# Improbable-AI/walk-these-ways

Hardware: NVIDIA H100
Metric: env_steps_per_s (higher is better)
Workload: dtype tf32

## Files before the change

### walk-these-ways_b200/csrc/gemm_tf32.cu

```cuda
#include <cuda_runtime.h>
#include <cuda.h>
#include <stdint.h>
#include <stdio.h>
#include <mutex>
#include <unordered_map>
#include <stdlib.h>
#include "../../include/go1_b200.h"
#include "wgmma_tf32.cuh"
#include "activation.cuh"

extern int go1_set_error(const char* m);
void go1_count_launch(int n);

namespace {

constexpr int BM = 128, BK = 32;
constexpr int NCONS = 8, EPI_G = 2;

__device__ __forceinline__ uint32_t smem_u32(const void* p) { return (uint32_t)__cvta_generic_to_shared(p); }

__device__ __forceinline__ void mbar_init(uint64_t* bar, uint32_t count) {
    asm volatile("mbarrier.init.shared::cta.b64 [%0], %1;" ::"r"(smem_u32(bar)), "r"(count));
}
__device__ __forceinline__ void mbar_expect_tx(uint64_t* bar, uint32_t bytes) {
    asm volatile("mbarrier.arrive.expect_tx.shared::cta.b64 _, [%0], %1;" ::"r"(smem_u32(bar)), "r"(bytes) : "memory");
}
__device__ __forceinline__ void mbar_wait(uint64_t* bar, uint32_t parity) {
    uint32_t done = 0;
    const uint32_t a = smem_u32(bar);
    while (!done) {
        asm volatile("{\n\t.reg .pred p;\n\tmbarrier.try_wait.parity.shared::cta.b64 p, [%1], %2;\n\tselp.u32 %0, 1, 0, p;\n\t}"
                     : "=r"(done) : "r"(a), "r"(parity) : "memory");
    }
}
__device__ __forceinline__ void mbar_arrive(uint64_t* bar) {
    asm volatile("mbarrier.arrive.shared::cta.b64 _, [%0];" ::"r"(smem_u32(bar)) : "memory");
}
__device__ __forceinline__ bool elect_one() {
    uint32_t pred = 0;
    asm volatile("{\n\t.reg .pred p;\n\telect.sync _|p, 0xffffffff;\n\tselp.u32 %0, 1, 0, p;\n\t}" : "=r"(pred));
    return pred != 0;
}
__device__ __forceinline__ void tma_load_2d(const CUtensorMap* map, uint64_t* bar, void* dst, int c0, int c1) {
    asm volatile("cp.async.bulk.tensor.2d.shared::cluster.global.mbarrier::complete_tx::bytes [%0], [%1, {%3, %4}], [%2];"
                 ::"r"(smem_u32(dst)), "l"(map), "r"(smem_u32(bar)), "r"(c0), "r"(c1) : "memory");
}
__device__ __forceinline__ void cons_sync() { asm volatile("bar.sync 1, 256;" ::: "memory"); }
__device__ __forceinline__ void wg_sync(int wgi) { asm volatile("bar.sync %0, 128;" ::"r"(2 + wgi) : "memory"); }
__device__ __forceinline__ void fence_async_smem() { asm volatile("fence.proxy.async.shared::cta;" ::: "memory"); }

template <int W>
__device__ __forceinline__ void transpose_tile(const float* __restrict__ raw, uint8_t* dst, const int ctid) {
#pragma unroll
    for (int it = 0; it < W * 8 / 256; it++) {
        const int idx = ctid + 256 * it;
        const int mn = idx % W, kq = idx / W;
        const float* r = raw + (size_t)(4 * kq) * W + mn;
        *reinterpret_cast<float4*>(dst + mn * 128 + ((kq ^ (mn & 7)) << 4)) = make_float4(r[0], r[W], r[2 * W], r[3 * W]);
    }
}

template <int NJ, typename F>
__device__ __forceinline__ void store_fragment(const float (&acc)[4 * NJ], uint8_t* tile, const int col_base, const int w, const int lane, F f) {
    const int rb = 16 * w + (lane >> 2);
#pragma unroll
    for (int j = 0; j < NJ; j++) {
        const int col = col_base + 8 * j + 2 * (lane & 3);
        uint8_t* p = tile + (size_t)(col >> 5) * (64 * 128) + rb * 128 + ((((col & 31) >> 2) ^ (rb & 7)) << 4) + (lane & 1) * 8;
        *reinterpret_cast<float2*>(p) = f(make_float2(acc[4 * j], acc[4 * j + 1]), col, 0);
        *reinterpret_cast<float2*>(p + 8 * 128) = f(make_float2(acc[4 * j + 2], acc[4 * j + 3]), col, 1);
    }
}


struct GemmArgs {
    float* C; const float* bias;
    int M, N, K, ldc, act, kind, accumulate, kb_per_split;
    const float* ex; const float* wex; const float* aux;
    int ldex, ldwex, nex, ldaux;
    int lead;
    int amn, bmn;
    int ct;
    float* colsum;
    const float* bx; const float* bwx; float* gwx; float* dx;
    int ldbx, ldbwx, ldgwx, lddx, nbx;
    int tma_store, tma_aux;
    float* Cg[4]; int nprob, tiles_per_prob;
};
constexpr int GEMM_MAXP = 4;
struct GemmMaps { CUtensorMap a[GEMM_MAXP], b[GEMM_MAXP]; };

struct EpiStage {
    uint8_t* out;
    const CUtensorMap* mapC;
    const uint8_t* aux;
};
__device__ __forceinline__ void tma_store_2d(const CUtensorMap* map, const void* src, int c0, int c1) {
    asm volatile("cp.async.bulk.tensor.2d.global.shared::cta.bulk_group [%0, {%2, %3}], [%1];"
                 ::"l"(map), "r"(smem_u32(src)), "r"(c0), "r"(c1) : "memory");
}

template <typename D>
__device__ __forceinline__ void epilogue_dact(const D dact, const GemmArgs& g, float (&v)[32], const int row, const int col0, const int ncols, const int lane,
                                              const float4 (&ypre)[8], const bool have_pre, const EpiStage& es) {
    const float* arow = g.aux + (size_t)row * g.ldaux + col0;
    if (es.aux) {
        const uint8_t* srow = es.aux + lane * 128;
#pragma unroll
        for (int j = 0; j < 8; j++) {
            const float4 y = *reinterpret_cast<const float4*>(srow + ((j ^ (lane & 7)) << 4));
            v[4 * j] *= dact(y.x); v[4 * j + 1] *= dact(y.y); v[4 * j + 2] *= dact(y.z); v[4 * j + 3] *= dact(y.w);
        }
    } else if (have_pre) {
#pragma unroll
        for (int j = 0; j < 8; j++) {
            const float4 y = ypre[j];
            v[4 * j] *= dact(y.x); v[4 * j + 1] *= dact(y.y); v[4 * j + 2] *= dact(y.z); v[4 * j + 3] *= dact(y.w);
        }
    } else if (ncols == 32 && (g.ldaux & 3) == 0 && ((((uintptr_t)g.aux) & 15) == 0) && ((col0 & 3) == 0)) {
#pragma unroll
        for (int j = 0; j < 8; j++) {
            const float4 y = __ldg(reinterpret_cast<const float4*>(arow) + j);
            v[4 * j] *= dact(y.x); v[4 * j + 1] *= dact(y.y); v[4 * j + 2] *= dact(y.z); v[4 * j + 3] *= dact(y.w);
        }
    } else {
#pragma unroll
        for (int j = 0; j < 32; j++) if (j < ncols) v[j] *= dact(__ldg(arow + j));
    }
}

__device__ __forceinline__ float transpose_reduce32(float (&sred)[32], const int lane) {
#pragma unroll
    for (int off = 16; off >= 1; off >>= 1) {
        const bool upper = (lane & off) != 0;
#pragma unroll
        for (int j = 0; j < off; j++) {
            const float send = upper ? sred[j] : sred[j + off];
            const float keep = upper ? sred[j + off] : sred[j];
            sred[j] = keep + __shfl_xor_sync(0xffffffffu, send, off);
        }
    }
    return sred[0];
}
// ... 92 lines not shown
                const float s = transpose_reduce32(sred, lane);
                if (lane < ncols) atomicAdd(g.gwx + (size_t)cjx * g.ldgwx + t, s);
                }
                if (g.dx) {
                    const float wl = lane < ncols ? __ldg(g.bwx + (size_t)cjx * g.ldbwx + t) : 0.f;
                    float acc = 0.f;
#pragma unroll
                    for (int j = 0; j < 32; j++) acc = fmaf(v[j], __shfl_sync(0xffffffffu, wl, j), acc);
                    if (row_ok) atomicAdd(g.dx + (size_t)row * g.lddx + t, acc);
                }
            }
        }
    }
    if (es.out) {
        if (g.ct) {
            __syncwarp();
#pragma unroll
            for (int j = 0; j < 32; j++)
                *reinterpret_cast<float*>(es.out + j * 128 + ((((lane >> 2) ^ (j & 7)) << 4) | ((lane & 3) << 2))) = v[j];
        } else {
            uint8_t* srow = es.out + lane * 128;
#pragma unroll
            for (int j = 0; j < 8; j++)
                *reinterpret_cast<float4*>(srow + ((j ^ (lane & 7)) << 4)) = make_float4(v[4 * j], v[4 * j + 1], v[4 * j + 2], v[4 * j + 3]);
        }
        asm volatile("fence.proxy.async.shared::cta;" ::: "memory");
        __syncwarp();
        if (lane == 0) {
            if (g.ct) tma_store_2d(es.mapC, es.out, row, col0);
            else tma_store_2d(es.mapC, es.out, col0, row);
            asm volatile("cp.async.bulk.commit_group;" ::: "memory");
        }
        return;
    }
    if (!row_ok) return;
    if (vec) {
#pragma unroll
        for (int j = 0; j < 8; j++) reinterpret_cast<float4*>(crow)[j] = make_float4(v[4 * j], v[4 * j + 1], v[4 * j + 2], v[4 * j + 3]);
    } else {
#pragma unroll
        for (int j = 0; j < 32; j++) if (j < ncols) crow[j] = v[j];
    }
}

__device__ __forceinline__ bool epilogue_prefetch(const GemmArgs& g, const int row, const int col0, const bool split, float4 (&ypre)[8]) {
    if (g.act != 2 || split || col0 + 32 > g.N || (g.ldaux & 3) != 0 || ((((uintptr_t)g.aux) & 15) != 0) || (col0 & 3) != 0) return false;
    const float4* arow = reinterpret_cast<const float4*>(g.aux + (size_t)(row < g.M ? row : 0) * g.ldaux + col0);
#pragma unroll
    for (int j = 0; j < 8; j++) ypre[j] = __ldg(arow + j);
    return true;
}

constexpr int X_BYTES = 65536;
template <int BN, bool ANYKIND>
__global__ void __launch_bounds__(32 * NCONS + 128, 1) gemm_tf32_wgmma(const __grid_constant__ GemmMaps gm,
                                                                      const __grid_constant__ CUtensorMap mapC, const __grid_constant__ CUtensorMap mapY, const GemmArgs g,
                                                                      const int tiles_m, const int tiles_n, const int total_tiles, const int stages) {
    constexpr int G = EPI_G;
    constexpr int A_BYTES = BM * BK * 4, STAGE_BYTES = (BM + BN) * BK * 4;
    constexpr int MAX_STAGES = 8;
    extern __shared__ __align__(1024) uint8_t smem_raw[];
    uint8_t* base = (uint8_t*)(((uintptr_t)smem_raw + 1023) & ~(uintptr_t)1023);
    uint8_t* ring = base;
    uint8_t* xreg = base + (size_t)stages * STAGE_BYTES;
    uint8_t* stage_aux = xreg + X_BYTES;
    uint64_t* full = (uint64_t*)(stage_aux + (g.tma_aux ? NCONS * 4096 : 0));
    uint64_t* empty = full + MAX_STAGES;
    uint64_t* aux_bar = empty + MAX_STAGES;

    const int warp = threadIdx.x >> 5, lane = threadIdx.x & 31;
    const int num_kb_total = (g.K + BK - 1) / BK;

    if (threadIdx.x == 0) {
        for (int p = 0; p < g.nprob; p++) {
            asm volatile("prefetch.tensormap [%0];" ::"l"(&gm.a[p]) : "memory");
            asm volatile("prefetch.tensormap [%0];" ::"l"(&gm.b[p]) : "memory");
        }
        if (g.tma_store) asm volatile("prefetch.tensormap [%0];" ::"l"(&mapC) : "memory");
        if (g.tma_aux) asm volatile("prefetch.tensormap [%0];" ::"l"(&mapY) : "memory");
        for (int s = 0; s < stages; s++) { mbar_init(&full[s], 1); mbar_init(&empty[s], NCONS); }
        for (int w = 0; w < NCONS; w++) mbar_init(&aux_bar[w], 1);
        asm volatile("fence.mbarrier_init.release.cluster;" ::: "memory");
    }
    __syncthreads();

    auto tile_coords = [&](int t, int& m0, int& n0, int& kb0, int& nkb) {
        if (g.nprob > 1) t %= g.tiles_per_prob;
        const int tn = t % tiles_n; t /= tiles_n;
        const int tm = t % tiles_m; const int z = t / tiles_m;
        m0 = tm * BM; n0 = tn * BN; kb0 = z * g.kb_per_split; nkb = min(g.kb_per_split, num_kb_total - kb0);
    };

    if (warp == NCONS) {
        if (elect_one()) {
            int s = 0, ph = 0;
            for (int t = blockIdx.x; t < total_tiles; t += gridDim.x) {
                int m0, n0, kb0, nkb; tile_coords(t, m0, n0, kb0, nkb);
                const int p = g.nprob > 1 ? t / g.tiles_per_prob : 0;
                const CUtensorMap* mapA = &gm.a[p];
                const CUtensorMap* mapB = &gm.b[p];
                for (int i = 0; i < nkb; i++) {
                    mbar_wait(&empty[s], ph ^ 1);
                    mbar_expect_tx(&full[s], STAGE_BYTES);
                    uint8_t* a = ring + (size_t)s * STAGE_BYTES;
                    uint8_t* b = a + A_BYTES;
                    if (g.amn) tma_load_2d(mapA, &full[s], a, m0, (kb0 + i) * BK);
                    else tma_load_2d(mapA, &full[s], a, (kb0 + i) * BK, m0);
                    if (g.bmn) tma_load_2d(mapB, &full[s], b, n0, (kb0 + i) * BK);
                    else tma_load_2d(mapB, &full[s], b, (kb0 + i) * BK, n0);
                    if (++s == stages) { s = 0; ph ^= 1; }
                }
            }
        }
        return;
    }
    if (warp > NCONS) return;

    const int wgi = warp >> 2, w = warp & 3, ctid = threadIdx.x;
    const int q = 2 * wgi + (w & 1), grp = w >> 1;
    const bool tr = g.amn || g.bmn;
    const bool split = g.kb_per_split < num_kb_total;
    const bool st_out = g.tma_store, st_aux = g.tma_aux;
    uint8_t* xwg = xreg + wgi * (X_BYTES / 2);
    uint8_t* my_aux = stage_aux + warp * 4096;
    uint64_t* my_bar = &aux_bar[warp];
    int pt = blockIdx.x, pc = grp - G;
    auto next_chunk = [&]() -> bool {
        for (;;) {
            pc += G;
            if (pc >= BN / 32) { pt += gridDim.x; pc = grp; }
            if (pt >= total_tiles) return false;
            if (pc < BN / 32 && (pt % tiles_n) * BN + 32 * pc < g.N) return true;
        }
    };
    auto request_aux = [&]() {
        if (next_chunk() && lane == 0) {
            int m0, n0, kb0, nkb; tile_coords(pt, m0, n0, kb0, nkb);
            mbar_expect_tx(my_bar, 4096);
            tma_load_2d(&mapY, my_bar, my_aux, n0 + 32 * pc, m0 + 32 * q);
        }
    };
    if (st_aux) request_aux();
    uint32_t aux_phase = 0;
    int s = 0, ph = 0;
    float acc[BN / 2];
    for (int t = blockIdx.x; t < total_tiles; t += gridDim.x) {
        int m0, n0, kb0, nkb; tile_coords(t, m0, n0, kb0, nkb);
        if (st_out && lane == 0) asm volatile("cp.async.bulk.wait_group.read 0;" ::: "memory");
        cons_sync();
        int prev = -1;
        for (int i = 0; i < nkb; i++) {
            mbar_wait(&full[s], ph);
            const uint8_t* a = ring + (size_t)s * STAGE_BYTES;
            const uint8_t* b = a + A_BYTES;
            if (tr) {
                if (g.amn) { uint8_t* ta = xreg + (i & 1) * A_BYTES; transpose_tile<BM>((const float*)a, ta, ctid); a = ta; }
                if (g.bmn) { uint8_t* tb = xreg + 2 * A_BYTES + (i & 1) * A_BYTES; transpose_tile<BN>((const float*)b, tb, ctid); b = tb; }
                if (prev >= 0) {
                    wg::wait<0>();
                    if (lane == 0) mbar_arrive(&empty[prev]);
                }
                fence_async_smem();
                cons_sync();
            }
            wg::fence();
            wg::mma_kblock<BN>(acc, a + (size_t)wgi * 64 * 128, b, i > 0);
            wg::commit();
            if (!tr && prev >= 0) {
                wg::wait<1>();
                if (lane == 0) mbar_arrive(&empty[prev]);
            }
            prev = s;
            if (++s == stages) { s = 0; ph ^= 1; }
        }
        wg::wait<0>();
        if (lane == 0) mbar_arrive(&empty[prev]);
        if (tr) cons_sync();

        const int row = m0 + 32 * q + lane;
        float* const Cbase = g.nprob > 1 ? g.Cg[t / g.tiles_per_prob] : g.C;
        float4 ypre[8];
        const bool have_pre = !st_aux && (grp < BN / 32) && epilogue_prefetch(g, row, n0 + 32 * grp, split, ypre);
        store_fragment<BN / 8>(acc, xwg, 0, w, lane, [](float2 v, int, int) { return v; });
        wg_sync(wgi);
#pragma unroll 1
        for (int c = grp; c < BN / 32; c += G) {
            if (n0 + 32 * c >= g.N) break;
            uint8_t* blk = xwg + (size_t)c * (64 * 128) + (w & 1) * 4096;
            uint32_t r[32];
            const uint8_t* srow = blk + lane * 128;
#pragma unroll
            for (int j = 0; j < 8; j++) {
                const uint4 x = *reinterpret_cast<const uint4*>(srow + ((j ^ (lane & 7)) << 4));
                r[4 * j] = x.x; r[4 * j + 1] = x.y; r[4 * j + 2] = x.z; r[4 * j + 3] = x.w;
            }
            EpiStage es;
            es.out = st_out ? blk : nullptr; es.mapC = &mapC; es.aux = st_aux ? my_aux : nullptr;
            if (st_aux) { mbar_wait(my_bar, aux_phase); aux_phase ^= 1; }
            epilogue_chunk<ANYKIND>(g, Cbase, r, row, n0 + 32 * c, split, lane, ypre, have_pre && c == grp, es);
            if (st_aux) { __syncwarp(); request_aux(); }
        }
    }
    if (st_out && lane == 0) asm volatile("cp.async.bulk.wait_group 0;" ::: "memory");
}

typedef CUresult (*EncodeTiledFn)(CUtensorMap*, CUtensorMapDataType, cuuint32_t, void*, const cuuint64_t*, const cuuint64_t*, const cuuint32_t*,
                                  const cuuint32_t*, CUtensorMapInterleave, CUtensorMapSwizzle, CUtensorMapL2promotion, CUtensorMapFloatOOBfill);
EncodeTiledFn g_encode = nullptr;
std::once_flag g_once;

int sm_count() {
    static int sms = 0;
    if (!sms) { int dev = 0; cudaGetDevice(&dev); cudaDeviceGetAttribute(&sms, cudaDevAttrMultiProcessorCount, dev); if (sms <= 0) sms = 132; }
    return sms;
}

int make_map_uncached(CUtensorMap* map, const float* ptr, int rows, int cols, int ld, int box_rows, int box_cols, CUtensorMapSwizzle swz);
struct MapKey { const float* ptr; int rows, cols, ld, box_rows, box_cols, swz; bool operator==(const MapKey& o) const { return ptr == o.ptr && rows == o.rows && cols == o.cols && ld == o.ld && box_rows == o.box_rows && box_cols == o.box_cols && swz == o.swz; } };
struct MapKeyHash { size_t operator()(const MapKey& k) const { size_t h = (size_t)k.ptr; h = h * 1000003u ^ (size_t)k.rows; h = h * 1000003u ^ (size_t)k.cols; h = h * 1000003u ^ (size_t)k.ld; h = h * 1000003u ^ (size_t)(k.box_rows * 8 + k.swz); h = h * 1000003u ^ (size_t)k.box_cols; return h; } };
std::unordered_map<MapKey, CUtensorMap, MapKeyHash> g_map_cache;
std::mutex g_map_mutex;
int make_map(CUtensorMap* map, const float* ptr, int rows, int cols, int ld, int box_rows, int box_cols = BK, CUtensorMapSwizzle swz = CU_TENSOR_MAP_SWIZZLE_128B) {
    const MapKey key{ptr, rows, cols, ld, box_rows, box_cols, (int)swz};
    {
        std::lock_guard<std::mutex> lk(g_map_mutex);
        auto it = g_map_cache.find(key);
        if (it != g_map_cache.end()) { *map = it->second; return 0; }
    }
    if (int e = make_map_uncached(map, ptr, rows, cols, ld, box_rows, box_cols, swz)) return e;
    std::lock_guard<std::mutex> lk(g_map_mutex);
    if (g_map_cache.size() > 8192) g_map_cache.clear();
    g_map_cache.emplace(key, *map);
    return 0;
}
int make_map_mn(CUtensorMap* map, const float* ptr, int k_rows, int mn_cols, int ld, int width) {
    return make_map(map, ptr, k_rows, mn_cols, ld, BK, width, CU_TENSOR_MAP_SWIZZLE_NONE);
}
int make_map_uncached(CUtensorMap* map, const float* ptr, int rows, int cols, int ld, int box_rows, int box_cols, CUtensorMapSwizzle swz) {
    std::call_once(g_once, [] {
        void* fn = nullptr;
        cudaDriverEntryPointQueryResult q;
        if (cudaGetDriverEntryPoint("cuTensorMapEncodeTiled", &fn, cudaEnableDefault, &q) == cudaSuccess && q == cudaDriverEntryPointSuccess) g_encode = (EncodeTiledFn)fn;
    });
    if (!g_encode) return go1_set_error("cuTensorMapEncodeTiled unavailable");
    cuuint64_t dims[2] = {(cuuint64_t)cols, (cuuint64_t)rows};
    cuuint64_t strides[1] = {(cuuint64_t)ld * 4};
    cuuint32_t box[2] = {(cuuint32_t)box_cols, (cuuint32_t)box_rows};
    cuuint32_t estr[2] = {1, 1};
    CUresult r = g_encode(map, CU_TENSOR_MAP_DATA_TYPE_FLOAT32, 2, (void*)ptr, dims, strides, box, estr, CU_TENSOR_MAP_INTERLEAVE_NONE,
                          swz, CU_TENSOR_MAP_L2_PROMOTION_L2_256B, CU_TENSOR_MAP_FLOAT_OOB_FILL_NONE);
    if (r != CUDA_SUCCESS) { char b[96]; snprintf(b, sizeof b, "cuTensorMapEncodeTiled failed (%d)", (int)r); return go1_set_error(b); }
    return 0;
}

int split_count(int tiles, int num_kb, int min_kb, int sms) {
    constexpr int SPLIT_TILE_KB = 4;
    int best = 1;
    long long best_cost = -1;
    for (int s = 1; s <= num_kb / (min_kb > 0 ? min_kb : 1); s++) {
        const int kb = (num_kb + s - 1) / s;
        if ((num_kb + kb - 1) / kb != s) continue;
        const long long cost = (long long)(((long long)tiles * s + sms - 1) / sms) * (kb + SPLIT_TILE_KB);
        if (best_cost < 0 || cost < best_cost) { best = s; best_cost = cost; }
    }
    return best;
}

__global__ void zero_strided(float* C, int ldc, int M, int N) {
    const size_t i = (size_t)blockIdx.x * blockDim.x + threadIdx.x;
    if (i >= (size_t)M * N) return;
    C[(i / N) * ldc + (i % N)] = 0.f;
}
__global__ void bias_act_strided(float* C, int ldc, const float* bias, int M, int N, int act, int kind) {
    const size_t i = (size_t)blockIdx.x * blockDim.x + threadIdx.x;
    if (i >= (size_t)M * N) return;
    float* c = C + (i / N) * ldc + (i % N);
    float v = *c;
    if (bias) v += bias[i % N];
    if (act == 1) { GO1_ACT_SWITCH(kind, KD, v = act_exact<KD>(v);) }
    *c = v;
}

template <int BN, bool ANYKIND>
int launch_gemm(const GemmMaps& gm, const CUtensorMap& mc, const CUtensorMap& my, GemmArgs& g, int splits, cudaStream_t st) {
    constexpr int STAGE_BYTES = (BM + BN) * BK * 4;
    const size_t staging = X_BYTES + (g.tma_aux ? (size_t)NCONS * 4096 : 0);
    const size_t fixed = staging + (2 * 8 + NCONS) * 8 + 16 + 1024;
    const size_t budget = 227 * 1024;
    int stages = (int)((budget - fixed) / STAGE_BYTES);
    if (stages > 8) stages = 8;
    if (stages < 2) return go1_set_error("go1_gemm impl=1: no room for the operand ring");
    const size_t smem = (size_t)stages * STAGE_BYTES + fixed;
    static bool configured = false;
    if (!configured) {
        cudaError_t e = cudaFuncSetAttribute(gemm_tf32_wgmma<BN, ANYKIND>, cudaFuncAttributeMaxDynamicSharedMemorySize, (int)budget);
        if (e != cudaSuccess) return go1_set_error(cudaGetErrorString(e));
        configured = true;
    }
    const int tiles_m = (g.M + BM - 1) / BM, tiles_n = (g.N + BN - 1) / BN;
    g.tiles_per_prob = tiles_m * tiles_n * splits;
    const int total = g.tiles_per_prob * (g.nprob > 1 ? g.nprob : 1);
    const int sms = sm_count();
    const int grid = total < sms ? total : sms;
    gemm_tf32_wgmma<BN, ANYKIND><<<grid, 32 * NCONS + 128, smem, st>>>(gm, mc, my, g, tiles_m, tiles_n, total, stages);
    go1_count_launch(1);
    return 0;
}

constexpr int TAIL_MAXP = 2, TAIL_HPW = 12, TAIL_BM = 64;
struct TailProb { const float* b2; const float* b3; const float* Wh; const float* bh; float* y3; float* out; int ldy3, ldout, nh, wh_row0; };
struct TailArgs { TailProb p[TAIL_MAXP]; int nprob, M, tiles_per_prob, tiles, kind; };
struct TailMaps { CUtensorMap x[TAIL_MAXP], w2[TAIL_MAXP], w3[TAIL_MAXP], y2[TAIL_MAXP]; };

template <int K1, int N2, int N3>
struct TailSmem {
    static constexpr int S1 = (N3 > 0) ? 2 : 3, S2 = (N3 > 0) ? 2 : 0;
    static constexpr int KB1 = K1 / BK, KB2 = N2 / BK;
    static constexpr int STAGE1 = (TAIL_BM + N2) * BK * 4;
    static constexpr int Y2TILE = KB2 * TAIL_BM * BK * 4;
    static constexpr int STAGE2 = (N3 > 0 ? N3 : 8) * BK * 4;
    static constexpr int NL = (N3 > 0) ? N3 : N2;
    static constexpr int PARAMS = (TAIL_MAXP * (N2 + N3) + 16 * NL + TAIL_MAXP * 16) * 4;
    static constexpr int HP = TAIL_HPW * TAIL_BM * 4;
    static constexpr int BARS = (2 * S1 + 2 * (S2 > 0 ? S2 : 1)) * 8 + 16;
    static constexpr int TOTAL = S1 * STAGE1 + Y2TILE + S2 * STAGE2 + PARAMS + HP + BARS + 1024;
};

template <int NJ>
__device__ __forceinline__ void head_partial(const float (&v)[4 * NJ], const float* wh, const int NL, const int nh, const int col_base, const int lane, float (&hp)[2][TAIL_HPW]) {
#pragma unroll
    for (int n = 0; n < TAIL_HPW; n++) {
        if (n < nh) {
            const float* wr = wh + n * NL + col_base + 2 * (lane & 3);
            float a0 = hp[0][n], a1 = hp[1][n];
#pragma unroll
            for (int j = 0; j < NJ; j++) {
                const float2 ww = *reinterpret_cast<const float2*>(wr + 8 * j);
                a0 = fmaf(v[4 * j], ww.x, a0); a0 = fmaf(v[4 * j + 1], ww.y, a0);
                a1 = fmaf(v[4 * j + 2], ww.x, a1); a1 = fmaf(v[4 * j + 3], ww.y, a1);
            }
            hp[0][n] = a0; hp[1][n] = a1;
        }
    }
}

template <int K1, int N2, int N3, bool ANYKIND>
__global__ void __launch_bounds__(32 * NCONS + 128, 1) mlp_tail_fwd_kernel(const __grid_constant__ TailMaps maps, const TailArgs g) {
    const int kind = ANYKIND ? g.kind : (int)GO1_ACT_ELU;
    using L = TailSmem<K1, N2, N3>;
    constexpr int S1 = L::S1, S2 = (L::S2 > 0 ? L::S2 : 1), KB1 = L::KB1, KB2 = L::KB2, STAGE1 = L::STAGE1, STAGE2 = L::STAGE2, NL = L::NL;
    constexpr int NH2 = N2 / 2, NH3 = (N3 > 0 ? N3 : 64) / 2;
    extern __shared__ __align__(1024) uint8_t smem_raw[];
    uint8_t* base = (uint8_t*)(((uintptr_t)smem_raw + 1023) & ~(uintptr_t)1023);
    uint8_t* r1 = base;
    uint8_t* y2t = r1 + S1 * STAGE1;
    uint8_t* r2 = y2t + L::Y2TILE;
    float* s_b2 = (float*)(r2 + L::S2 * STAGE2);
// ... 130 lines not shown
            if (n < pr.nh) {
#pragma unroll
                for (int r = 0; r < 2; r++) {
                    float a = hp[r][n];
                    a += __shfl_xor_sync(0xffffffffu, a, 1);
                    a += __shfl_xor_sync(0xffffffffu, a, 2);
                    hp[r][n] = a;
                }
                if (wgi == 1 && (lane & 3) == 0) { s_hp[n * TAIL_BM + rA] = hp[0][n]; s_hp[n * TAIL_BM + rA + 8] = hp[1][n]; }
            }
        }
        cons_sync();
        if (wgi == 0 && (lane & 3) == 0) {
            const float* bh = s_bh + p * 16;
#pragma unroll
            for (int n = 0; n < TAIL_HPW; n++) {
                if (n < pr.nh) {
                    if (ok0) pr.out[(size_t)(m0 + rA) * pr.ldout + n] = hp[0][n] + s_hp[n * TAIL_BM + rA] + bh[n];
                    if (ok1) pr.out[(size_t)(m0 + rA + 8) * pr.ldout + n] = hp[1][n] + s_hp[n * TAIL_BM + rA + 8] + bh[n];
                }
            }
        }
        if (lane == 0) asm volatile("cp.async.bulk.wait_group.read 0;" ::: "memory");
        cons_sync();
    }
    if (lane == 0) asm volatile("cp.async.bulk.wait_group 0;" ::: "memory");
}

template <int K1, int N2, int N3, bool ANYKIND>
int launch_tail(const TailMaps& maps, const TailArgs& g, cudaStream_t st) {
    using L = TailSmem<K1, N2, N3>;
    static_assert(L::TOTAL <= 227 * 1024, "fused tail: shared memory budget");
    const size_t smem = L::TOTAL;
    static bool configured = false;
    if (!configured) {
        cudaError_t e = cudaFuncSetAttribute(mlp_tail_fwd_kernel<K1, N2, N3, ANYKIND>, cudaFuncAttributeMaxDynamicSharedMemorySize, (int)smem);
        if (e != cudaSuccess) return go1_set_error(cudaGetErrorString(e));
        configured = true;
    }
    const int sms = sm_count();
    const int grid = g.tiles < sms ? g.tiles : sms;
    mlp_tail_fwd_kernel<K1, N2, N3, ANYKIND><<<grid, 32 * NCONS + 128, smem, st>>>(maps, g);
    go1_count_launch(1);
    return 0;
}

}

#include <vector>
static bool g_time_on = false;
static std::vector<cudaEvent_t> g_time_events;
static size_t g_time_used = 0;
static double g_time_flop = 0.0;
struct TimeRec { int M, N, K, amn, bmn, act, nex, splits, kern, colsum; };
static std::vector<TimeRec> g_time_recs;
static cudaEvent_t timing_event() {
    if (g_time_used == g_time_events.size()) { cudaEvent_t e; cudaEventCreate(&e); g_time_events.push_back(e); }
    return g_time_events[g_time_used++];
}
extern "C" int go1_gemm_timing(int on, double* total_ms, double* total_flop, long long* launches) {
    if (on) { g_time_on = true; g_time_used = 0; g_time_flop = 0.0; g_time_recs.clear(); return 0; }
    g_time_on = false;
    double ms = 0.0;
    FILE* csv = getenv("GO1_GEMM_TIMING_CSV") ? fopen(getenv("GO1_GEMM_TIMING_CSV"), "w") : nullptr;
    if (csv) fprintf(csv, "M,N,K,a_mn_major,b_mn_major,act,num_extra,splits,kernel,colsum,us\n");
    for (size_t i = 0; i + 1 < g_time_used; i += 2) {
        if (cudaEventSynchronize(g_time_events[i + 1]) != cudaSuccess) return go1_set_error("go1_gemm_timing: event sync failed");
        float t = 0.f;
        if (cudaEventElapsedTime(&t, g_time_events[i], g_time_events[i + 1]) != cudaSuccess) return go1_set_error("go1_gemm_timing: elapsed time failed");
        ms += t;
        if (csv && i / 2 < g_time_recs.size()) {
            const TimeRec& r = g_time_recs[i / 2];
            fprintf(csv, "%d,%d,%d,%d,%d,%d,%d,%d,%s,%d,%.2f\n", r.M, r.N, r.K, r.amn, r.bmn, r.act, r.nex, r.splits,
                    r.kern >= 1000 ? (r.kern == 1003 ? "tail3" : "tail2") : (r.kern == 128 ? "p128" : (r.kern == 64 ? "p64" : "p32")), r.colsum, 1e3 * t);
        }
    }
    if (csv) fclose(csv);
    if (total_ms) *total_ms = ms;
    if (total_flop) *total_flop = g_time_flop;
    if (launches) *launches = (long long)(g_time_used / 2);
    return 0;
}

static int gemm_tf32_impl(int transA, int transB, int M, int N, int K, int nprob, const float* const* As, int lda, const float* const* Bs, int ldb,
                          float* const* Cs, int ldc, const Go1GemmEpilogue* ep, cudaStream_t st) {
    float* Cm = Cs[0];
    const float* bias = ep->bias; const int act = ep->act, accumulate = ep->accumulate;
    if (act < 0 || act > 2) return go1_set_error("go1_gemm_ex: act must be 0, 1 or 2");
    if (!go1_act_kind_ok(ep->act_kind)) return go1_set_error("go1_gemm_ex: unknown activation kind (Go1Activation)");
    const int amn = transA ? 1 : 0, bmn = transB ? 0 : 1;
    for (int p = 0; p < nprob; p++)
        if ((lda & 3) || (ldb & 3) || (((uintptr_t)As[p] | (uintptr_t)Bs[p]) & 15) || !Cs[p])
            return go1_set_error("go1_gemm impl=1: A/B must be 16-byte aligned with row strides that are multiples of 4 floats (TMA)");
    GemmArgs g;
    g.nprob = nprob; g.tiles_per_prob = 0;
    for (int p = 0; p < GEMM_MAXP; p++) g.Cg[p] = Cs[p < nprob ? p : 0];
    g.C = Cm; g.bias = bias; g.M = M; g.N = N; g.K = K; g.ldc = ldc; g.act = act; g.kind = ep->act_kind; g.accumulate = accumulate;
    g.ex = ep->extra; g.ldex = ep->ld_extra; g.wex = ep->w_extra; g.ldwex = ep->ld_w_extra; g.nex = ep->extra ? ep->num_extra : 0;
    g.aux = ep->dact_y; g.ldaux = ep->ld_dact_y;
    g.amn = amn; g.bmn = bmn; g.lead = ep->lead_cols; g.colsum = ep->colsum; g.ct = ep->store_transposed ? 1 : 0;
    g.nbx = ep->num_bwd_extra; g.bx = ep->bwd_extra; g.bwx = ep->bwd_w_extra; g.gwx = ep->g_w_extra; g.dx = ep->d_extra;
    g.ldbx = ep->ld_bwd_extra; g.ldbwx = ep->ld_bwd_w_extra; g.ldgwx = ep->ld_g_w_extra; g.lddx = ep->ld_d_extra;
    if (g.nbx < 0 || g.nbx > 4 || (g.nbx > 0 && ((g.gwx && !g.bx) || (!g.gwx && !g.dx) || (g.dx && !g.bwx)))) return go1_set_error("go1_gemm_ex: bad fused trailing-input backward arguments");
    if (g.nex < 0 || g.nex > 4) return go1_set_error("go1_gemm_ex: num_extra must be 0..4");
    if (act == 2 && !g.aux) return go1_set_error("go1_gemm_ex: act 2 needs dact_y");
    if (g.ct && (nprob != 1 || accumulate || M < 32 || (ldc & 3) || (((uintptr_t)Cm) & 15)))
        return go1_set_error("go1_gemm_ex: store_transposed needs M >= 32, no accumulate and a 16-byte aligned C with ldc a multiple of 4");
    const int num_kb = (K + BK - 1) / BK;
    constexpr int SPLIT_MIN_KB = 16;
    const int BN = (N > 64) ? 128 : (N > 32 ? 64 : 32);
    const int tiles = ((M + BM - 1) / BM) * ((N + BN - 1) / BN) * nprob;
    const bool plain = g.nex == 0 && act != 2 && g.lead <= 0 && !g.colsum && g.nbx == 0 && !g.ct;
    const int splits = plain ? split_count(tiles, num_kb, SPLIT_MIN_KB, sm_count()) : 1;
    g.kb_per_split = (num_kb + splits - 1) / splits;
    GemmMaps gm;
    for (int p = 0; p < nprob; p++) {
        if (int e = amn ? make_map_mn(&gm.a[p], As[p], K, M, lda, BM) : make_map(&gm.a[p], As[p], M, K, lda, BM)) return e;
        if (int e = bmn ? make_map_mn(&gm.b[p], Bs[p], K, N, ldb, BN) : make_map(&gm.b[p], Bs[p], N, K, ldb, BN)) return e;
    }
    for (int p = nprob; p < GEMM_MAXP; p++) { gm.a[p] = gm.a[0]; gm.b[p] = gm.b[0]; }
    const CUtensorMap& ma = gm.a[0];
    if (splits > 1) {
        if (!accumulate)
            for (int p = 0; p < nprob; p++) { const size_t tot = (size_t)M * N; zero_strided<<<(unsigned)((tot + 255) / 256), 256, 0, st>>>(Cs[p], ldc, M, N); go1_count_launch(1); }
        g.bias = nullptr; g.act = 0;
    }
    cudaStreamCaptureStatus cap = cudaStreamCaptureStatusNone;
    const bool timed = g_time_on && cudaStreamIsCapturing(st, &cap) == cudaSuccess && cap == cudaStreamCaptureStatusNone;
    if (timed) {
        cudaEventRecord(timing_event(), st); g_time_flop += 2.0 * (double)M * (double)N * (double)K * nprob;
        g_time_recs.push_back({M * nprob, N, K, amn, bmn, act, g.nex, splits, BN, g.colsum ? 1 : 0});
    }
    int e;
    CUtensorMap mc = ma, my = ma;
    g.tma_store = g.tma_aux = 0;
    if (nprob == 1 && splits == 1 && !accumulate && (g.ct ? M : N) >= 32 && (ldc & 3) == 0 && (((uintptr_t)Cm) & 15) == 0) {
        if (int e2 = g.ct ? make_map(&mc, Cm, N, M, ldc, 32) : make_map(&mc, Cm, M, N, ldc, 32)) return e2;
        g.tma_store = 1;
        if (g.act == 2 && (g.ldaux & 3) == 0 && (((uintptr_t)g.aux) & 15) == 0) {
            if (int e2 = make_map(&my, g.aux, M, N, g.ldaux, 32)) return e2;
            g.tma_aux = 1;
        }
    }
    const bool any = g.act != 0 && g.kind != GO1_ACT_ELU;
    if (BN == 128) e = any ? launch_gemm<128, true>(gm, mc, my, g, splits, st) : launch_gemm<128, false>(gm, mc, my, g, splits, st);
    else if (BN == 64) e = any ? launch_gemm<64, true>(gm, mc, my, g, splits, st) : launch_gemm<64, false>(gm, mc, my, g, splits, st);
    else e = any ? launch_gemm<32, true>(gm, mc, my, g, splits, st) : launch_gemm<32, false>(gm, mc, my, g, splits, st);
    if (e) return e;
    if (splits > 1 && (bias || act))
        for (int p = 0; p < nprob; p++) { const size_t tot = (size_t)M * N; bias_act_strided<<<(unsigned)((tot + 255) / 256), 256, 0, st>>>(Cs[p], ldc, bias, M, N, act, ep->act_kind); go1_count_launch(1); }
    if (timed) cudaEventRecord(timing_event(), st);
    cudaError_t ce = cudaGetLastError();
    if (ce != cudaSuccess) return go1_set_error(cudaGetErrorString(ce));
    return 0;
}

extern "C" int go1_gemm_tf32(int transA, int transB, int M, int N, int K, const float* A, int lda, const float* B, int ldb,
                             float* Cm, int ldc, const Go1GemmEpilogue* ep, cudaStream_t st) {
    return gemm_tf32_impl(transA, transB, M, N, K, 1, &A, lda, &B, ldb, &Cm, ldc, ep, st);
}
extern "C" int go1_gemm_grouped(int transA, int transB, int M, int N, int K, int nprob, const float* const* A, int lda, const float* const* B, int ldb,
                                float* const* C, int ldc, int accumulate, void* stream) {
    if (!A || !B || !C || nprob < 1 || nprob > GEMM_MAXP || M <= 0 || N <= 0 || K <= 0) return go1_set_error("go1_gemm_grouped: 1..4 problems");
    Go1GemmEpilogue ep = {};
    ep.accumulate = accumulate;
    return gemm_tf32_impl(transA, transB, M, N, K, nprob, A, lda, B, ldb, C, ldc, &ep, (cudaStream_t)stream);
}

__global__ void transpose_kernel(const float* __restrict__ src, int lds, float* __restrict__ dst, int ldd, int rows, int cols) {
    __shared__ float t[32][33];
    const int c0 = blockIdx.x * 32, r0 = blockIdx.y * 32;
    for (int i = threadIdx.y; i < 32; i += 8) {
        const int r = r0 + i, c = c0 + threadIdx.x;
        t[i][threadIdx.x] = (r < rows && c < cols) ? src[(size_t)r * lds + c] : 0.f;
    }
    __syncthreads();
    for (int i = threadIdx.y; i < 32; i += 8) {
        const int c = c0 + i, r = r0 + threadIdx.x;
        if (c < cols && r < rows) dst[(size_t)c * ldd + r] = t[threadIdx.x][i];
    }
}
extern "C" int go1_transpose(const float* src, int lds, float* dst, int ldd, int rows, int cols, void* stream) {
    if (!src || !dst || rows <= 0 || cols <= 0 || lds < cols || ldd < rows) return go1_set_error("go1_transpose: bad arguments");
    dim3 grid((cols + 31) / 32, (rows + 31) / 32);
    transpose_kernel<<<grid, dim3(32, 8), 0, (cudaStream_t)stream>>>(src, lds, dst, ldd, rows, cols);
    go1_count_launch(1);
    cudaError_t ce = cudaGetLastError();
    if (ce != cudaSuccess) return go1_set_error(cudaGetErrorString(ce));
    return 0;
}


extern "C" int go1_mlp_tail_forward_grouped(const Go1TailProblem* probs, int nprob, int M, int K1, int N2, int N3, void* stream) {
    cudaStream_t st = (cudaStream_t)stream;
    if (!probs || nprob < 1 || nprob > TAIL_MAXP || M <= 0) return go1_set_error("go1_mlp_tail_forward: 1 or 2 problems of the same shape");
    const bool shape_a = (K1 == 512 && N2 == 256 && N3 == 128), shape_b = (K1 == 256 && N2 == 128 && N3 == 0);
    if (!shape_a && !shape_b) return go1_set_error("go1_mlp_tail_forward: supported tails are 512-256-128-head and 256-128-head");
    TailMaps maps;
    TailArgs g;
    g.nprob = nprob; g.M = M; g.tiles_per_prob = (M + TAIL_BM - 1) / TAIL_BM; g.tiles = g.tiles_per_prob * nprob;
    g.kind = probs[0].act_kind;
    if (!go1_act_kind_ok(g.kind)) return go1_set_error("go1_mlp_tail_forward: unknown activation kind (Go1Activation)");
    int rows = 0;
    for (int p = 0; p < nprob; p++) {
        const Go1TailProblem& q = probs[p];
        if (q.act_kind != g.kind) return go1_set_error("go1_mlp_tail_forward: the problems of one launch share their activation kind");
        if (!q.x || !q.W2 || !q.y2 || !q.Wh || !q.out || q.nh < 1 || q.nh > TAIL_HPW || q.ldout < q.nh) return go1_set_error("go1_mlp_tail_forward: bad arguments (head width 1..12)");
        if (N3 > 0 && (!q.W3 || !q.y3)) return go1_set_error("go1_mlp_tail_forward: the three-layer tail needs W3 / y3");
        if ((q.ldx & 3) || (q.ldy2 & 3) || (N3 > 0 && (q.ldy3 & 3)) ||
            ((((uintptr_t)q.x | (uintptr_t)q.W2 | (uintptr_t)q.y2 | (uintptr_t)(N3 > 0 ? (const void*)q.W3 : (const void*)q.W2) |
               (uintptr_t)(N3 > 0 ? (const void*)q.y3 : (const void*)q.y2)) & 15) != 0))
            return go1_set_error("go1_mlp_tail_forward: operands must be 16-byte aligned with row strides that are multiples of 4 floats");
        if (int e = make_map(&maps.x[p], q.x, M, K1, q.ldx, TAIL_BM)) return e;
        if (int e = make_map(&maps.w2[p], q.W2, N2, K1, K1, N2)) return e;
        if (N3 > 0) { if (int e = make_map(&maps.w3[p], q.W3, N3, N2, N2, N3)) return e; } else maps.w3[p] = maps.w2[p];
        if (int e = make_map(&maps.y2[p], q.y2, M, N2, q.ldy2, 32)) return e;
        TailProb& d = g.p[p];
        d.b2 = q.b2; d.b3 = q.b3; d.Wh = q.Wh; d.bh = q.bh; d.y3 = q.y3; d.out = q.out; d.ldy3 = q.ldy3; d.ldout = q.ldout; d.nh = q.nh; d.wh_row0 = rows;
        rows += q.nh;
    }
    if (rows > 16) return go1_set_error("go1_mlp_tail_forward: the head rows of all problems must fit 16");
    for (int p = nprob; p < TAIL_MAXP; p++) { maps.x[p] = maps.x[0]; maps.w2[p] = maps.w2[0]; maps.w3[p] = maps.w3[0]; maps.y2[p] = maps.y2[0]; g.p[p] = g.p[0]; }
    cudaStreamCaptureStatus cap = cudaStreamCaptureStatusNone;
    const bool timed = g_time_on && cudaStreamIsCapturing(st, &cap) == cudaSuccess && cap == cudaStreamCaptureStatusNone;
    if (timed) {
        cudaEventRecord(timing_event(), st);
        double fl = 0.0;
        for (int p = 0; p < nprob; p++) fl += 2.0 * (double)M * ((double)K1 * N2 + (double)N2 * N3 + (double)(N3 > 0 ? N3 : N2) * probs[p].nh);
        g_time_flop += fl;
        g_time_recs.push_back({M * nprob, N2, K1, 0, 0, 1, 0, 1, shape_a ? 1003 : 1002, 0});
    }
    int e;
    if (g.kind == GO1_ACT_ELU) e = shape_a ? launch_tail<512, 256, 128, false>(maps, g, st) : launch_tail<256, 128, 0, false>(maps, g, st);
    else e = shape_a ? launch_tail<512, 256, 128, true>(maps, g, st) : launch_tail<256, 128, 0, true>(maps, g, st);
    if (e) return e;
    if (timed) cudaEventRecord(timing_event(), st);
    cudaError_t ce = cudaGetLastError();
    if (ce != cudaSuccess) return go1_set_error(cudaGetErrorString(ce));
    return 0;
}
extern "C" int go1_mlp_tail_forward(const float* x, int ldx, int M, int K1, const float* W2, const float* b2, int N2, float* y2, int ldy2,
                                    const float* W3, const float* b3, int N3, float* y3, int ldy3, const float* Wh, const float* bh, int nh,
                                    float* out, int ldout, void* stream) {
    Go1TailProblem q = {};
    q.x = x; q.ldx = ldx; q.W2 = W2; q.b2 = b2; q.y2 = y2; q.ldy2 = ldy2; q.W3 = W3; q.b3 = b3; q.y3 = y3; q.ldy3 = ldy3; q.Wh = Wh; q.bh = bh; q.nh = nh; q.out = out; q.ldout = ldout;
    return go1_mlp_tail_forward_grouped(&q, 1, M, K1, N2, N3, stream);
}
```

Baseline: 1.528 million.

## Pair CTAs in clusters and multicast the shared operand tile via TMA

Adds a 2-CTA cluster variant of the persistent TF32 WGMMA GEMM. Paired CTAs work on adjacent tiles that share one operand, and each CTA loads half of that shared tile with TMA multicast into both CTAs' shared memory. Empty barriers are released across the cluster so both consumers must finish before a slot is refilled. The goal is to cut L2/global operand traffic for non-transposed, single-problem BN=128 GEMMs. The cost is cross-CTA synchronisation coupling and occupancy limited by how many clusters fit.

```diff
diff --git a/walk-these-ways_b200/csrc/gemm_tf32.cu b/walk-these-ways_b200/csrc/gemm_tf32.cu
--- a/walk-these-ways_b200/csrc/gemm_tf32.cu
+++ b/walk-these-ways_b200/csrc/gemm_tf32.cu
@@ -44,6 +44,23 @@
 __device__ __forceinline__ void tma_load_2d(const CUtensorMap* map, uint64_t* bar, void* dst, int c0, int c1) {
     asm volatile("cp.async.bulk.tensor.2d.shared::cluster.global.mbarrier::complete_tx::bytes [%0], [%1, {%3, %4}], [%2];"
                  ::"r"(smem_u32(dst)), "l"(map), "r"(smem_u32(bar)), "r"(c0), "r"(c1) : "memory");
+}
+__device__ __forceinline__ void tma_load_2d_multicast(const CUtensorMap* map, uint64_t* bar, void* dst, int c0, int c1, uint16_t cta_mask) {
+    asm volatile("cp.async.bulk.tensor.2d.shared::cluster.global.mbarrier::complete_tx::bytes.multicast::cluster [%0], [%1, {%3, %4}], [%2], %5;"
+                 ::"r"(smem_u32(dst)), "l"(map), "r"(smem_u32(bar)), "r"(c0), "r"(c1), "h"(cta_mask) : "memory");
+}
+__device__ __forceinline__ uint32_t cluster_ctarank() {
+    uint32_t r;
+    asm("mov.u32 %0, %%cluster_ctarank;" : "=r"(r));
+    return r;
+}
+__device__ __forceinline__ void cluster_sync() {
+    asm volatile("barrier.cluster.arrive.release;\n\tbarrier.cluster.wait.acquire;" ::: "memory");
+}
+__device__ __forceinline__ void mbar_arrive_cluster(uint64_t* bar, uint32_t rank) {
+    uint32_t remote;
+    asm volatile("mapa.shared::cluster.u32 %0, %1, %2;" : "=r"(remote) : "r"(smem_u32(bar)), "r"(rank));
+    asm volatile("mbarrier.arrive.shared::cluster.b64 _, [%0];" ::"r"(remote) : "memory");
 }
 __device__ __forceinline__ void cons_sync() { asm volatile("bar.sync 1, 256;" ::: "memory"); }
 __device__ __forceinline__ void wg_sync(int wgi) { asm volatile("bar.sync %0, 128;" ::"r"(2 + wgi) : "memory"); }
@@ -88,7 +105,7 @@
     float* Cg[4]; int nprob, tiles_per_prob;
 };
 constexpr int GEMM_MAXP = 4;
-struct GemmMaps { CUtensorMap a[GEMM_MAXP], b[GEMM_MAXP]; };
+struct GemmMaps { CUtensorMap a[GEMM_MAXP], b[GEMM_MAXP], half; };
 
 struct EpiStage {
     uint8_t* out;
@@ -287,10 +304,11 @@
 }
 
 constexpr int X_BYTES = 65536;
-template <int BN, bool ANYKIND>
+template <int BN, bool ANYKIND, int CL>
 __global__ void __launch_bounds__(32 * NCONS + 128, 1) gemm_tf32_wgmma(const __grid_constant__ GemmMaps gm,
                                                                       const __grid_constant__ CUtensorMap mapC, const __grid_constant__ CUtensorMap mapY, const GemmArgs g,
                                                                       const int tiles_m, const int tiles_n, const int total_tiles, const int stages) {
+    static_assert(CL == 1 || (CL == 2 && BN == BM), "CTA pairs share 128-row operand boxes");
     constexpr int G = EPI_G;
     constexpr int A_BYTES = BM * BK * 4, STAGE_BYTES = (BM + BN) * BK * 4;
     constexpr int MAX_STAGES = 8;
@@ -313,14 +331,27 @@
         }
         if (g.tma_store) asm volatile("prefetch.tensormap [%0];" ::"l"(&mapC) : "memory");
         if (g.tma_aux) asm volatile("prefetch.tensormap [%0];" ::"l"(&mapY) : "memory");
-        for (int s = 0; s < stages; s++) { mbar_init(&full[s], 1); mbar_init(&empty[s], NCONS); }
+        if (CL > 1) asm volatile("prefetch.tensormap [%0];" ::"l"(&gm.half) : "memory");
+        for (int s = 0; s < stages; s++) { mbar_init(&full[s], 1); mbar_init(&empty[s], CL * NCONS); }
         for (int w = 0; w < NCONS; w++) mbar_init(&aux_bar[w], 1);
         asm volatile("fence.mbarrier_init.release.cluster;" ::: "memory");
     }
-    __syncthreads();
-
+    if (CL > 1) cluster_sync();
+    else __syncthreads();
+
+    const int npt = total_tiles / CL;
+    auto first = [] { return (int)blockIdx.x / CL; };
+    auto step = [] { return (int)gridDim.x / CL; };
+    auto rank = [] { return CL > 1 ? cluster_ctarank() : 0u; };
+    auto pair_n = [&] { return (tiles_n & 1) == 0; };
+    auto cta_tile = [&](int pt) -> int {
+        if (CL == 1) return pt;
+        if (pair_n()) return 2 * pt + (int)rank();
+        const int tn = pt % tiles_n, r = pt / tiles_n, hm = tiles_m / 2;
+        return ((r / hm) * tiles_m + 2 * (r % hm) + (int)rank()) * tiles_n + tn;
+    };
     auto tile_coords = [&](int t, int& m0, int& n0, int& kb0, int& nkb) {
-        if (g.nprob > 1) t %= g.tiles_per_prob;
+        if (CL == 1 && g.nprob > 1) t %= g.tiles_per_prob;
         const int tn = t % tiles_n; t /= tiles_n;
         const int tm = t % tiles_m; const int z = t / tiles_m;
         m0 = tm * BM; n0 = tn * BN; kb0 = z * g.kb_per_split; nkb = min(g.kb_per_split, num_kb_total - kb0);
@@ -329,9 +360,10 @@
     if (warp == NCONS) {
         if (elect_one()) {
             int s = 0, ph = 0;
-            for (int t = blockIdx.x; t < total_tiles; t += gridDim.x) {
+            for (int pt = first(); pt < npt; pt += step()) {
+                const int t = cta_tile(pt);
                 int m0, n0, kb0, nkb; tile_coords(t, m0, n0, kb0, nkb);
-                const int p = g.nprob > 1 ? t / g.tiles_per_prob : 0;
+                const int p = CL == 1 && g.nprob > 1 ? t / g.tiles_per_prob : 0;
                 const CUtensorMap* mapA = &gm.a[p];
                 const CUtensorMap* mapB = &gm.b[p];
                 for (int i = 0; i < nkb; i++) {
@@ -339,38 +371,59 @@
                     mbar_expect_tx(&full[s], STAGE_BYTES);
                     uint8_t* a = ring + (size_t)s * STAGE_BYTES;
                     uint8_t* b = a + A_BYTES;
-                    if (g.amn) tma_load_2d(mapA, &full[s], a, m0, (kb0 + i) * BK);
-                    else tma_load_2d(mapA, &full[s], a, (kb0 + i) * BK, m0);
-                    if (g.bmn) tma_load_2d(mapB, &full[s], b, n0, (kb0 + i) * BK);
-                    else tma_load_2d(mapB, &full[s], b, (kb0 + i) * BK, n0);
+                    if (CL > 1) {
+                        const int kc = (kb0 + i) * BK;
+                        if (pair_n()) {
+                            tma_load_2d_multicast(&gm.half, &full[s], a + rank() * (A_BYTES / 2), kc, m0 + (int)rank() * (BM / 2), 0x3);
+                            tma_load_2d(mapB, &full[s], b, kc, n0);
+                        } else {
+                            tma_load_2d(mapA, &full[s], a, kc, m0);
+                            tma_load_2d_multicast(&gm.half, &full[s], b + rank() * (A_BYTES / 2), kc, n0 + (int)rank() * (BN / 2), 0x3);
+                        }
+                    } else {
+                        if (g.amn) tma_load_2d(mapA, &full[s], a, m0, (kb0 + i) * BK);
+                        else tma_load_2d(mapA, &full[s], a, (kb0 + i) * BK, m0);
+                        if (g.bmn) tma_load_2d(mapB, &full[s], b, n0, (kb0 + i) * BK);
+                        else tma_load_2d(mapB, &full[s], b, (kb0 + i) * BK, n0);
+                    }
                     if (++s == stages) { s = 0; ph ^= 1; }
                 }
             }
         }
+        if (CL > 1) cluster_sync();
         return;
     }
-    if (warp > NCONS) return;
+    if (warp > NCONS) {
+        if (CL > 1) cluster_sync();
+        return;
+    }
 
     const int wgi = warp >> 2, w = warp & 3, ctid = threadIdx.x;
     const int q = 2 * wgi + (w & 1), grp = w >> 1;
-    const bool tr = g.amn || g.bmn;
+    const bool tr = CL == 1 && (g.amn || g.bmn);
     const bool split = g.kb_per_split < num_kb_total;
-    const bool st_out = g.tma_store, st_aux = g.tma_aux;
+    const bool st_out = g.tma_store, st_aux = CL == 1 && g.tma_aux;
     uint8_t* xwg = xreg + wgi * (X_BYTES / 2);
     uint8_t* my_aux = stage_aux + warp * 4096;
     uint64_t* my_bar = &aux_bar[warp];
-    int pt = blockIdx.x, pc = grp - G;
+    int pt = first(), pc = grp - G;
     auto next_chunk = [&]() -> bool {
         for (;;) {
             pc += G;
-            if (pc >= BN / 32) { pt += gridDim.x; pc = grp; }
-            if (pt >= total_tiles) return false;
-            if (pc < BN / 32 && (pt % tiles_n) * BN + 32 * pc < g.N) return true;
+            if (pc >= BN / 32) { pt += step(); pc = grp; }
+            if (pt >= npt) return false;
+            if (pc < BN / 32 && (cta_tile(pt) % tiles_n) * BN + 32 * pc < g.N) return true;
+        }
+    };
+    auto release = [&](int s) {
+        if (lane == 0) {
+            mbar_arrive(&empty[s]);
+            if (CL > 1) mbar_arrive_cluster(&empty[s], rank() ^ 1);
         }
     };
     auto request_aux = [&]() {
         if (next_chunk() && lane == 0) {
-            int m0, n0, kb0, nkb; tile_coords(pt, m0, n0, kb0, nkb);
+            int m0, n0, kb0, nkb; tile_coords(cta_tile(pt), m0, n0, kb0, nkb);
             mbar_expect_tx(my_bar, 4096);
             tma_load_2d(&mapY, my_bar, my_aux, n0 + 32 * pc, m0 + 32 * q);
         }
@@ -379,7 +432,8 @@
     uint32_t aux_phase = 0;
     int s = 0, ph = 0;
     float acc[BN / 2];
-    for (int t = blockIdx.x; t < total_tiles; t += gridDim.x) {
+    for (int tp = first(); tp < npt; tp += step()) {
+        const int t = cta_tile(tp);
         int m0, n0, kb0, nkb; tile_coords(t, m0, n0, kb0, nkb);
         if (st_out && lane == 0) asm volatile("cp.async.bulk.wait_group.read 0;" ::: "memory");
         cons_sync();
@@ -393,7 +447,7 @@
                 if (g.bmn) { uint8_t* tb = xreg + 2 * A_BYTES + (i & 1) * A_BYTES; transpose_tile<BN>((const float*)b, tb, ctid); b = tb; }
                 if (prev >= 0) {
                     wg::wait<0>();
-                    if (lane == 0) mbar_arrive(&empty[prev]);
+                    release(prev);
                 }
                 fence_async_smem();
                 cons_sync();
@@ -403,19 +457,19 @@
             wg::commit();
             if (!tr && prev >= 0) {
                 wg::wait<1>();
-                if (lane == 0) mbar_arrive(&empty[prev]);
+                release(prev);
             }
             prev = s;
             if (++s == stages) { s = 0; ph ^= 1; }
         }
         wg::wait<0>();
-        if (lane == 0) mbar_arrive(&empty[prev]);
+        release(prev);
         if (tr) cons_sync();
 
         const int row = m0 + 32 * q + lane;
-        float* const Cbase = g.nprob > 1 ? g.Cg[t / g.tiles_per_prob] : g.C;
+        float* const Cbase = CL == 1 && g.nprob > 1 ? g.Cg[t / g.tiles_per_prob] : g.C;
         float4 ypre[8];
-        const bool have_pre = !st_aux && (grp < BN / 32) && epilogue_prefetch(g, row, n0 + 32 * grp, split, ypre);
+        const bool have_pre = CL == 1 && !st_aux && (grp < BN / 32) && epilogue_prefetch(g, row, n0 + 32 * grp, split, ypre);
         store_fragment<BN / 8>(acc, xwg, 0, w, lane, [](float2 v, int, int) { return v; });
         wg_sync(wgi);
 #pragma unroll 1
@@ -437,6 +491,7 @@
         }
     }
     if (st_out && lane == 0) asm volatile("cp.async.bulk.wait_group 0;" ::: "memory");
+    if (CL > 1) cluster_sync();
 }
 
 typedef CUresult (*EncodeTiledFn)(CUtensorMap*, CUtensorMapDataType, cuuint32_t, void*, const cuuint64_t*, const cuuint64_t*, const cuuint32_t*,
@@ -516,7 +571,7 @@
     *c = v;
 }
 
-template <int BN, bool ANYKIND>
+template <int BN, bool ANYKIND, int CL>
 int launch_gemm(const GemmMaps& gm, const CUtensorMap& mc, const CUtensorMap& my, GemmArgs& g, int splits, cudaStream_t st) {
     constexpr int STAGE_BYTES = (BM + BN) * BK * 4;
     const size_t staging = X_BYTES + (g.tma_aux ? (size_t)NCONS * 4096 : 0);
@@ -526,18 +581,39 @@
     if (stages > 8) stages = 8;
     if (stages < 2) return go1_set_error("go1_gemm impl=1: no room for the operand ring");
     const size_t smem = (size_t)stages * STAGE_BYTES + fixed;
-    static bool configured = false;
-    if (!configured) {
-        cudaError_t e = cudaFuncSetAttribute(gemm_tf32_wgmma<BN, ANYKIND>, cudaFuncAttributeMaxDynamicSharedMemorySize, (int)budget);
-        if (e != cudaSuccess) return go1_set_error(cudaGetErrorString(e));
-        configured = true;
-    }
+    auto kernel = gemm_tf32_wgmma<BN, ANYKIND, CL>;
     const int tiles_m = (g.M + BM - 1) / BM, tiles_n = (g.N + BN - 1) / BN;
     g.tiles_per_prob = tiles_m * tiles_n * splits;
     const int total = g.tiles_per_prob * (g.nprob > 1 ? g.nprob : 1);
-    const int sms = sm_count();
-    const int grid = total < sms ? total : sms;
-    gemm_tf32_wgmma<BN, ANYKIND><<<grid, 32 * NCONS + 128, smem, st>>>(gm, mc, my, g, tiles_m, tiles_n, total, stages);
+    cudaLaunchConfig_t cfg = {};
+    cudaLaunchAttribute attr[1];
+    attr[0].id = cudaLaunchAttributeClusterDimension;
+    attr[0].val.clusterDim.x = CL; attr[0].val.clusterDim.y = 1; attr[0].val.clusterDim.z = 1;
+    cfg.blockDim = dim3(32 * NCONS + 128); cfg.dynamicSmemBytes = smem; cfg.stream = st;
+    cfg.attrs = attr; cfg.numAttrs = 1;
+    static bool configured = false;
+    static int slots = 0;
+    if (!configured) {
+        cudaError_t e = cudaFuncSetAttribute(kernel, cudaFuncAttributeMaxDynamicSharedMemorySize, (int)budget);
+        if (e != cudaSuccess) return go1_set_error(cudaGetErrorString(e));
+        slots = sm_count();
+        if (CL > 1) {
+            cfg.gridDim = dim3(CL * sm_count());
+            int clusters = 0;
+            e = cudaOccupancyMaxActiveClusters(&clusters, kernel, &cfg);
+            if (e != cudaSuccess) return go1_set_error(cudaGetErrorString(e));
+            if (clusters < 1) return go1_set_error("go1_gemm impl=1: no CTA pair of the persistent GEMM fits a GPC");
+            slots = clusters;
+        }
+        configured = true;
+    }
+    const int units = total / CL;
+    cfg.gridDim = dim3(CL * (units < slots ? units : slots));
+    if (CL == 1) kernel<<<cfg.gridDim, cfg.blockDim, smem, st>>>(gm, mc, my, g, tiles_m, tiles_n, total, stages);
+    else {
+        cudaError_t e = cudaLaunchKernelEx(&cfg, kernel, gm, mc, my, g, tiles_m, tiles_n, total, stages);
+        if (e != cudaSuccess) return go1_set_error(cudaGetErrorString(e));
+    }
     go1_count_launch(1);
     return 0;
 }
@@ -774,7 +850,7 @@
 static std::vector<cudaEvent_t> g_time_events;
 static size_t g_time_used = 0;
 static double g_time_flop = 0.0;
-struct TimeRec { int M, N, K, amn, bmn, act, nex, splits, kern, colsum; };
+struct TimeRec { int M, N, K, amn, bmn, act, nex, splits, kern, colsum, cluster; };
 static std::vector<TimeRec> g_time_recs;
 static cudaEvent_t timing_event() {
     if (g_time_used == g_time_events.size()) { cudaEvent_t e; cudaEventCreate(&e); g_time_events.push_back(e); }
@@ -794,7 +870,8 @@
         if (csv && i / 2 < g_time_recs.size()) {
             const TimeRec& r = g_time_recs[i / 2];
             fprintf(csv, "%d,%d,%d,%d,%d,%d,%d,%d,%s,%d,%.2f\n", r.M, r.N, r.K, r.amn, r.bmn, r.act, r.nex, r.splits,
-                    r.kern >= 1000 ? (r.kern == 1003 ? "tail3" : "tail2") : (r.kern == 128 ? "p128" : (r.kern == 64 ? "p64" : "p32")), r.colsum, 1e3 * t);
+                    r.kern >= 1000 ? (r.kern == 1003 ? "tail3" : "tail2") : (r.kern == 128 ? (r.cluster == 2 ? "p128c2" : "p128") : (r.kern == 64 ? "p64" : "p32")),
+                    r.colsum, 1e3 * t);
         }
     }
     if (csv) fclose(csv);
@@ -842,6 +919,12 @@
     }
     for (int p = nprob; p < GEMM_MAXP; p++) { gm.a[p] = gm.a[0]; gm.b[p] = gm.b[0]; }
     const CUtensorMap& ma = gm.a[0];
+    const int tiles_m = (M + BM - 1) / BM, tiles_n = (N + BN - 1) / BN;
+    const int cluster = (!amn && !bmn && nprob == 1 && act != 2 && BN == 128 && (tiles_n % 2 == 0 || tiles_m % 2 == 0)) ? 2 : 1;
+    gm.half = ma;
+    if (cluster == 2) {
+        if (int e = tiles_n % 2 == 0 ? make_map(&gm.half, As[0], M, K, lda, BM / 2) : make_map(&gm.half, Bs[0], N, K, ldb, BN / 2)) return e;
+    }
     if (splits > 1) {
         if (!accumulate)
             for (int p = 0; p < nprob; p++) { const size_t tot = (size_t)M * N; zero_strided<<<(unsigned)((tot + 255) / 256), 256, 0, st>>>(Cs[p], ldc, M, N); go1_count_launch(1); }
@@ -851,7 +934,7 @@
     const bool timed = g_time_on && cudaStreamIsCapturing(st, &cap) == cudaSuccess && cap == cudaStreamCaptureStatusNone;
     if (timed) {
         cudaEventRecord(timing_event(), st); g_time_flop += 2.0 * (double)M * (double)N * (double)K * nprob;
-        g_time_recs.push_back({M * nprob, N, K, amn, bmn, act, g.nex, splits, BN, g.colsum ? 1 : 0});
+        g_time_recs.push_back({M * nprob, N, K, amn, bmn, act, g.nex, splits, BN, g.colsum ? 1 : 0, cluster});
     }
     int e;
     CUtensorMap mc = ma, my = ma;
@@ -865,9 +948,10 @@
         }
     }
     const bool any = g.act != 0 && g.kind != GO1_ACT_ELU;
-    if (BN == 128) e = any ? launch_gemm<128, true>(gm, mc, my, g, splits, st) : launch_gemm<128, false>(gm, mc, my, g, splits, st);
-    else if (BN == 64) e = any ? launch_gemm<64, true>(gm, mc, my, g, splits, st) : launch_gemm<64, false>(gm, mc, my, g, splits, st);
-    else e = any ? launch_gemm<32, true>(gm, mc, my, g, splits, st) : launch_gemm<32, false>(gm, mc, my, g, splits, st);
+    if (cluster == 2) e = any ? launch_gemm<128, true, 2>(gm, mc, my, g, splits, st) : launch_gemm<128, false, 2>(gm, mc, my, g, splits, st);
+    else if (BN == 128) e = any ? launch_gemm<128, true, 1>(gm, mc, my, g, splits, st) : launch_gemm<128, false, 1>(gm, mc, my, g, splits, st);
+    else if (BN == 64) e = any ? launch_gemm<64, true, 1>(gm, mc, my, g, splits, st) : launch_gemm<64, false, 1>(gm, mc, my, g, splits, st);
+    else e = any ? launch_gemm<32, true, 1>(gm, mc, my, g, splits, st) : launch_gemm<32, false, 1>(gm, mc, my, g, splits, st);
     if (e) return e;
     if (splits > 1 && (bias || act))
         for (int p = 0; p < nprob; p++) { const size_t tot = (size_t)M * N; bias_act_strided<<<(unsigned)((tot + 255) / 256), 256, 0, st>>>(Cs[p], ldc, bias, M, N, act, ep->act_kind); go1_count_launch(1); }
@@ -950,7 +1034,7 @@
         double fl = 0.0;
         for (int p = 0; p < nprob; p++) fl += 2.0 * (double)M * ((double)K1 * N2 + (double)N2 * N3 + (double)(N3 > 0 ? N3 : N2) * probs[p].nh);
         g_time_flop += fl;
-        g_time_recs.push_back({M * nprob, N2, K1, 0, 0, 1, 0, 1, shape_a ? 1003 : 1002, 0});
+        g_time_recs.push_back({M * nprob, N2, K1, 0, 0, 1, 0, 1, shape_a ? 1003 : 1002, 0, 1});
     }
     int e;
     if (g.kind == GO1_ACT_ELU) e = shape_a ? launch_tail<512, 256, 128, false>(maps, g, st) : launch_tail<256, 128, 0, false>(maps, g, st);
```

New measurement: 1.643 million (median of 6 runs). 1.08x the previous value.
